# automl/RoBO

Measured on NVIDIA H100. Metric: EI evals/sec (GP N=4096, D=16, fp64), higher is better.
Workload: dtype f64

## Files before the change

robo_b200/csrc/gpk_api.cu:

```cuda
#include <algorithm>
#include <cmath>
#include <cstdarg>
#include <cstdio>
#include <cstring>
#include <cstdlib>
#include <dlfcn.h>
#include <string>
#include <vector>

#include "gpk_gemm.cuh"
#include "gpk_kernels.cuh"
#include "gpk_diag16.cuh"
#include "gpk_ozaki.cuh"
#include "gpk_de.cuh"
#include "gpk_lbfgs.cuh"
#include "gpk_cmaes.cuh"
#include "gpk_direct.cuh"
#include "gpk_es.cuh"
#include "gpk_esmc.cuh"
#include "gpk_rs.cuh"
#include "gpk_hyper.cuh"
#include "gpk_blr.cuh"
#include "gpk_rf.cuh"

// ... 7 lines not shown
    void* p = nullptr;
    size_t cap = 0;
};

}

struct gpk_handle {
    int device = 0;
    cudaStream_t stream = nullptr;
    cudaStream_t own_stream = nullptr;
    cudaStream_t side_stream = nullptr;
    std::vector<cudaEvent_t> ev_panel, ev_rest;
    int ozaki = 1;
    DevBuf oz_Pq, oz_Kq, oz_Kq2, oz_eP, oz_emax, oz_pmu2;
    int oz_last_variant = 0;
    int oz_cluster = 4;
    int oz_map_cs = 0;
    int oz_max_clusters[5] = {0, 0, 0, 0, 0};
    int oz_persist = 3;
    int oz_grid = 0;
    DevBuf oz_probe;
    long oz_linv_serial = -1;
    long linv_serial = 0;
    int oz_emax_host = 0;
    long oz_rows = 0, oz_rows2 = 0;
    CUtensorMap mapOzP, mapOzK, mapOzK2;
    double oz_launches = 0;
    int n_sm = 0;
    char err[1024] = {0};
    int loader = LOADER_TMA_WS;
    long chunk = 16384;
    bool chunk_user = false;
    int diag_prof = 0;
    DevBuf dprof;

    int n = 0, d = 0, NP = 0, nb = 0;
// ... 273 lines not shown
            attr[0].val.clusterDim.x = (unsigned)cs;
            attr[0].val.clusterDim.y = 1;
            attr[0].val.clusterDim.z = 1;
            cfg.attrs = attr;
            cfg.numAttrs = 1;
            int n = 0;
            CK(cudaOccupancyMaxActiveClusters(&n, gpk_oz_vargemm_kernel, &cfg));
            if (n < 1) { set_err(h, "no cluster of %d int8 contraction CTAs fits on this device", cs); return GPK_CUDA_ERROR; }
            h->oz_max_clusters[cs] = n;
        }
    }
    *out = h->oz_max_clusters[cs];
    return GPK_OK;
}

int launch_oz_contraction(gpk_handle* h, const CUtensorMap& mapP, const CUtensorMap& mapK, int nb, long rows_padded,
                          long NP, long rows, const int* eP, int eK, double* part_ssq, long ldpart) {
    OzArgs o;
    o.nb = nb; o.ncb = (int)(rows_padded / OZ_TN); o.NP = (int)NP; o.rows = (int)rows;
    const int cs = h->oz_cluster;
    o.group = (int)std::min<long>(512, std::max<long>(4, ((long)24 << 20) / ((long)OZ_TN * NP * OZ_S))) / cs * cs;
    o.eP = eP; o.eK = eK;
    o.part_ssq = part_ssq; o.ldpart = ldpart;
    const int persist = h->oz_persist == 3 ? (nb <= 32 ? 1 : 0) : h->oz_persist;
    const int tiles = o.nb * o.ncb;
    int grid = tiles;
    if (persist == 1) {
        int nclusters = 0, rc;
        if ((rc = oz_max_clusters(h, cs, &nclusters))) return rc;
        if (h->oz_grid > 0) nclusters = std::min(nclusters, h->oz_grid);
        grid = cs * std::min(tiles / cs, nclusters);
    }
    h->oz_last_variant = 1 + (persist == 1 ? 8 : 0) + (cs == 2 ? 16 : cs == 4 ? 32 : 0);
    CK(launch_oz(gpk_oz_vargemm_kernel, (unsigned)grid, cs, (size_t)OZ_SMEM, h->stream, mapP, mapK, o));
    CKL();
    return GPK_OK;
}

template <int EPI, int MI = 8>
int launch_gemm(gpk_handle* h, const CUtensorMap& mA, const CUtensorMap& mB, const GemmArgs& a, int njobs,
                cudaStream_t stream = nullptr, bool pdl = false) {
    if (njobs <= 0) return GPK_OK;
    if (stream == nullptr) stream = h->stream;
    if (pdl && h->loader != LOADER_CPASYNC && MI == 2) {
        CK(launch_pdl(gpk_gemm_nt_kernel<EPI, LOADER_TMA, MI>, dim3(njobs), dim3(GEMM_THREADS),
                      (size_t)gemm_smem_bytes(LOADER_TMA, MI), stream, mA, mB, a));
// ... 375 lines not shown
        const int lowest = -100000;
        CK(cudaMemcpyAsync(h->oz_emax.p, &lowest, 4, cudaMemcpyHostToDevice, h->stream));
        gpk_oz_rowexp_kernel<<<(unsigned)NP, 256, 0, h->stream>>>(ptr<double>(h->P), NP, (int)NP, ptr<int>(h->oz_eP), ptr<int>(h->oz_emax));
        CKL();
        gpk_oz_split_kernel<<<(unsigned)((NP * NP + 255) / 256), 256, 0, h->stream>>>(ptr<double>(h->P), NP, NP, ptr<int>(h->oz_eP), 0,
                                                                                   ptr<int8_t>(h->oz_Pq), NP * NP);
        CKL();
        if ((rc = ensure_alpha(h))) return rc;
        CK(cudaMemcpyAsync(&h->oz_emax_host, h->oz_emax.p, 4, cudaMemcpyDeviceToHost, h->stream));
        CK(cudaStreamSynchronize(h->stream));
        h->oz_map_cs = 0;
        h->oz_linv_serial = h->linv_serial;
    }
    if (h->oz_map_cs != h->oz_cluster) {
        int rc;
        if ((rc = make_oz_map(h, &h->mapOzP, h->oz_Pq.p, (long)OZ_S * NP, NP, OZ_TM / h->oz_cluster))) return rc;
        h->oz_map_cs = h->oz_cluster;
    }
    *usable = h->oz_emax_host <= OZ_MAX_EXP;
    return GPK_OK;
}

long chunk_rows(const gpk_handle* h) {
    if (h->chunk_user) return h->chunk;
    long c = ((1L << 26) / std::max(h->NP, 128)) / BM * BM;
    return std::min<long>(65536, std::max<long>(4096, c));
}

struct Feeder {
    virtual int ready(long lo, long hi, cudaStream_t st) = 0;
    virtual ~Feeder() {}
// ... 11 lines not shown
              long index_offset = 0, bool reset = true, long global_base = 0, Feeder* feeder = nullptr) {
    if (h->blr)
        return blr_score(h, dX, m, kind, eta, par, d_out, d_mu, d_var, d_best, d_nneg, index_offset, reset, global_base,
                         feeder);
    if (h->rf)
        return rf_score(h, dX, m, kind, eta, par, d_out, d_mu, d_var, d_best, d_nneg, index_offset, reset, global_base,
                        feeder);
    int rc = build_linv(h);
    if (rc) return rc;
    const long NP = h->NP;
    const long cap = std::min<long>(chunk_rows(h), round_up(std::max<long>(m, 1), BM));
    if ((rc = ensure_score_scratch(h, cap))) return rc;
    bool use_oz = false;
    if (m >= 2048 && (rc = prepare_ozaki(h, &use_oz))) return rc;
    int oz_eK = 0;
    if (use_oz) {
        if ((rc = ensure(h, h->oz_Kq, (size_t)OZ_S * cap * NP))) return rc;
        if (h->overlap && (rc = ensure(h, h->oz_Kq2, (size_t)OZ_S * cap * NP))) return rc;
        if ((rc = make_oz_map(h, &h->mapOzK, h->oz_Kq.p, (long)OZ_S * cap, NP, OZ_TN))) return rc;
        if (h->overlap && (rc = make_oz_map(h, &h->mapOzK2, h->oz_Kq2.p, (long)OZ_S * cap, NP, OZ_TN))) return rc;
        if (h->overlap && (rc = ensure(h, h->oz_pmu2, (size_t)h->nb * cap * 8))) return rc;
        oz_eK = oz_exponent(h->spec.amp);
    }
    if (d_best == nullptr) d_best = ptr<BestPair>(h->best);
    if (d_nneg == nullptr) d_nneg = ptr<unsigned long long>(h->nneg);
    if (reset) {
        CK(cudaMemsetAsync(d_best, 0xFF, sizeof(BestPair), h->stream));
        CK(cudaMemsetAsync(d_nneg, 0, 8, h->stream));
    }
    CK(cudaEventRecord(h->ev[6], h->stream));
    const int nchunks = (int)((m + cap - 1) / cap);
    const bool pipelined = h->overlap && nchunks > 1;
    if (pipelined) {
        while ((int)h->ev_cov.size() < nchunks) {
            cudaEvent_t e1, e2;
// ... 21 lines not shown
            if (frc) return frc;
        }
        const double* lo = h->has_bounds ? ptr<double>(h->lower) : nullptr;
        const double* up = h->has_bounds ? ptr<double>(h->upper) : nullptr;
        if (!use_oz)
            return launch_cov_tiles(h, st, train_operand(h), NP, h->n, dX + base * h->d, h->d, mc, mcp, lo, up,
                                    second ? ptr<double>(h->Kstar2) : ptr<double>(h->Kstar), NP, 0, small);
        CUtensorMap map;
        int mrc = make_cov_map(h, &map, (void*)train_operand(h), h->spec.n_terms, NP);
        if (mrc) return mrc;
        int8_t* qdst = second ? ptr<int8_t>(h->oz_Kq2) : ptr<int8_t>(h->oz_Kq);
        double* pmu = second ? ptr<double>(h->oz_pmu2) : ptr<double>(h->part_mu);
        const int gx = (int)(NP / 128);
        if (small)
            gpk_cov_oz_kernel<4><<<(unsigned)(gx * (mcp / 16)), 256, cov_oz_smem_bytes(h->spec.n_terms, 4), st>>>(
                map, h->spec, h->n, dX + base * h->d, h->d, mc, lo, up, ptr<double>(h->alpha), oz_eK, qdst, NP, cap * NP, pmu, cap, gx);
        else
            gpk_cov_oz_kernel<8><<<(unsigned)(gx * (mcp / 32)), 256, cov_oz_smem_bytes(h->spec.n_terms, 8), st>>>(
                map, h->spec, h->n, dX + base * h->d, h->d, mc, lo, up, ptr<double>(h->alpha), oz_eK, qdst, NP, cap * NP, pmu, cap, gx);
        CKL();
        return GPK_OK;
    };
    if (pipelined) {
        CK(cudaEventRecord(h->ev_order, h->stream));
        CK(cudaStreamWaitEvent(h->side_stream, h->ev_order, 0));
        if ((rc = launch_cov(0, h->side_stream, false))) return rc;
        CK(cudaEventRecord(h->ev_cov[0], h->side_stream));
    }
    for (int ci = 0; ci < nchunks; ++ci) {
        const long base = (long)ci * cap;
        const long mc = std::min(cap, m - base);
        const long mcp = round_up(mc, BM);
        const bool last = ci == nchunks - 1;
        if (last) CK(cudaEventRecord(h->ev[8], h->stream));
// ... 10 lines not shown
        const bool second = pipelined && (ci & 1);
        GemmArgs a;
        memset(&a, 0, sizeof(a));
        a.A = ptr<double>(h->P); a.lda = NP;
        a.B = second ? ptr<double>(h->Kstar2) : ptr<double>(h->Kstar); a.ldb = NP;
        a.alpha = 1.0;
        a.job_mode = JOBS_VARIANCE;
        a.nb = h->nb; a.mcb = (int)(mcp / BN);
        a.z = ptr<double>(h->Kbuf) + NP * NP;
        a.part_mu = ptr<double>(h->part_mu);
        a.part_ssq = ptr<double>(h->part_ssq);
        a.ldpart = cap;
        if (last) CK(cudaEventRecord(h->ev[10], h->stream));
        CK(cudaEventRecord(h->ev_g0[ci], h->stream));
        if (use_oz) {
            if ((rc = launch_oz_contraction(h, h->mapOzP, second ? h->mapOzK2 : h->mapOzK, h->nb, mcp, NP, cap,
                                            ptr<int>(h->oz_eP), oz_eK, a.part_ssq, a.ldpart)))
                return rc;
            h->oz_launches += 1;
        } else if ((rc = launch_gemm<EPI_COLREDUCE>(h, h->mapP, second ? h->mapKs2 : h->mapKs, a, h->nb * a.mcb))) return rc;
        CK(cudaEventRecord(h->ev_g1[ci], h->stream));
        if (last) CK(cudaEventRecord(h->ev[11], h->stream));
        if (pipelined && !use_oz) CK(cudaEventRecord(h->ev_gemm[ci], h->stream));
        h->launches_var += 1;
        h->last_chunk_rows = mcp;
        FinishArgs f;
        memset(&f, 0, sizeof(f));
        f.part_mu = ptr<double>(h->part_mu); f.part_ssq = ptr<double>(h->part_ssq);
        f.ldpart = cap; f.nparts = h->nb; f.m = mc; f.base = global_base + index_offset + base;
        f.kss = h->spec.amp; f.mean = h->mean;
        f.norm_out = h->norm_out; f.y_mean = h->y_mean; f.y_std = h->y_std;
// ... 381 lines not shown
    if (cudaMallocHost((void**)&h->pin, 64) != cudaSuccess) { delete h; return GPK_CUDA_ERROR; }
    if (get_encode_fn() == nullptr) h->loader = LOADER_CPASYNC;
    *out = h;
    return GPK_OK;
}

int gpk_destroy(gpk_handle* h) {
    if (!h) return GPK_OK;
    cudaSetDevice(h->device);
    cudaStreamSynchronize(h->stream);
    gpk_comm_destroy(h);
    if (h->ev_multi) cudaEventDestroy(h->ev_multi);
    DevBuf* bufs[] = {&h->Xrow, &h->Xt, &h->y, &h->Kbuf, &h->P, &h->Q, &h->W, &h->lower, &h->upper, &h->logdet_part,
                      &h->scal, &h->status, &h->jobs, &h->cand, &h->Kstar, &h->Kstar2, &h->cand2, &h->part_mu, &h->part_ssq, &h->out_mu,
                      &h->out_var, &h->out_acq, &h->block_best, &h->best, &h->nneg, &h->Vt, &h->cov, &h->XsT,
                      &h->tmpjobs, &h->alpha, &h->tmp1, &h->tmp2, &h->tmp3, &h->dprof, &h->Xts, &h->oz_Pq, &h->oz_Kq, &h->oz_Kq2, &h->oz_eP, &h->oz_emax, &h->oz_pmu2, &h->oz_probe,
                      &h->multi_cand, &h->multi_A, &h->multi_B, &h->multi_out, &h->multi_bb, &h->gather, &h->best_global,
                      &h->de_pop, &h->de_trial, &h->de_param, &h->de_E, &h->de_small, &h->de_sort, &h->lb_buf, &h->cma_buf, &h->dir_buf, &h->ep_buf, &h->es_state, &h->es_U, &h->es_work, &h->es_in, &h->mc_state, &h->mc_buf, &h->mc_stat, &h->fab_in, &h->rs_buf, &h->hy_buf,
                      &h->blr_data, &h->blr_post, &h->blr_work, &h->blr_bb,
                      &h->rf_data, &h->rf_work, &h->rf_nodes, &h->rf_bb};
    for (DevBuf* b : bufs)
        if (b->p) cudaFree(b->p);
    if (h->ev_ok)
        for (int i = 0; i < 16; ++i) cudaEventDestroy(h->ev[i]);
    if (h->ev_order) cudaEventDestroy(h->ev_order);
    for (int i = 0; i < 2; ++i)
        if (h->stage[i]) cudaFreeHost(h->stage[i]);
    for (cudaEvent_t e : h->ev_panel) cudaEventDestroy(e);
    for (cudaEvent_t e : h->ev_rest) cudaEventDestroy(e);
    for (cudaEvent_t e : h->ev_cov) cudaEventDestroy(e);
    for (cudaEvent_t e : h->ev_g0) cudaEventDestroy(e);
// ... 1471 lines not shown
    CK(cudaMemcpyAsync(z, ptr<double>(h->Kbuf) + (long)h->NP * h->NP, (size_t)h->n * 8, cudaMemcpyDeviceToHost, h->stream));
    CK(cudaStreamSynchronize(h->stream));
    return GPK_OK;
}

int gpk_oz_contract(gpk_handle* h, const double* P, int n, const double* Ks, long m, double amp, double* part_ssq,
                    int* eP, int* eK) {
    if (!h) return GPK_BAD_ARG;
    if (!P || !Ks || !part_ssq || !eP || !eK || n <= 0 || m <= 0 || !(amp > 0.0) || !std::isfinite(amp))
        BAD("gpk_oz_contract: bad arguments");
    const long NP = round_up(n, OZ_TM), MP = round_up(m, OZ_TM), nb = NP / OZ_TM;
    if (NP > 16384) BAD("gpk_oz_contract: n = %d pads to %ld > 16384 (the int32 level sums hold K <= 16384)", n, NP);
    for (long i = 0; i < m * (long)n; ++i)
        if (!(std::fabs(Ks[i]) <= amp)) BAD("gpk_oz_contract: |Ks| exceeds amp at entry %ld", i);
    CK(cudaSetDevice(h->device));
    const size_t oK = (size_t)NP * NP * 8, oPq = oK + (size_t)MP * NP * 8, oKq = oPq + (size_t)OZ_S * NP * NP;
    const size_t opart = oKq + (size_t)OZ_S * MP * NP, oe = opart + (size_t)nb * MP * 8, oemax = oe + (size_t)NP * 4;
    int rc;
    if ((rc = ensure(h, h->oz_probe, oemax + 4))) return rc;
    char* b = (char*)h->oz_probe.p;
    double* dP = (double*)b;
    double* dK = (double*)(b + oK);
    int8_t* dPq = (int8_t*)(b + oPq);
    int8_t* dKq = (int8_t*)(b + oKq);
    double* dpart = (double*)(b + opart);
    int* de = (int*)(b + oe);
    cudaStream_t st = h->stream;
    CK(cudaMemsetAsync(dP, 0, (size_t)NP * NP * 8, st));
    CK(cudaMemcpy2DAsync(dP, (size_t)NP * 8, P, (size_t)n * 8, (size_t)n * 8, (size_t)n, cudaMemcpyHostToDevice, st));
    CK(cudaMemsetAsync(dK, 0, (size_t)MP * NP * 8, st));
    CK(cudaMemcpy2DAsync(dK, (size_t)NP * 8, Ks, (size_t)n * 8, (size_t)n * 8, (size_t)m, cudaMemcpyHostToDevice, st));
    CK(cudaMemsetAsync(b + oemax, 0, 4, st));
    CK(cudaMemsetAsync(dpart, 0xFF, (size_t)nb * MP * 8, st));
    gpk_oz_rowexp_kernel<<<(unsigned)NP, 256, 0, st>>>(dP, NP, (int)NP, de, (int*)(b + oemax));
    CKL();
    gpk_oz_split_kernel<<<(unsigned)((NP * NP + 255) / 256), 256, 0, st>>>(dP, NP, NP, de, 0, dPq, NP * NP);
    CKL();
    const int ek = oz_exponent(amp);
    gpk_oz_split_kernel<<<(unsigned)((MP * NP + 255) / 256), 256, 0, st>>>(dK, MP, NP, nullptr, ek, dKq, MP * NP);
    CKL();
    CUtensorMap mapP, mapK;
    if ((rc = make_oz_map(h, &mapP, dPq, (long)OZ_S * NP, NP, OZ_TM / h->oz_cluster))) return rc;
    if ((rc = make_oz_map(h, &mapK, dKq, (long)OZ_S * MP, NP, OZ_TN))) return rc;
    if ((rc = launch_oz_contraction(h, mapP, mapK, (int)nb, MP, NP, MP, de, ek, dpart, MP))) return rc;
    CK(cudaMemcpy2DAsync(part_ssq, (size_t)m * 8, dpart, (size_t)MP * 8, (size_t)m * 8, (size_t)nb, cudaMemcpyDeviceToHost, st));
    CK(cudaMemcpyAsync(eP, de, (size_t)n * 4, cudaMemcpyDeviceToHost, st));
    CK(cudaStreamSynchronize(st));
    *eK = ek;
    return GPK_OK;
}

int gpk_ep_joint_min(gpk_handle* h, const double* mu, const double* V, int nb, double* logP, double* dlogPdMu,
                     double* dlogPdSigma, double* dlogPdMudMu, int* sweeps) {
    if (!h) return GPK_BAD_ARG;
    if (!mu || !V || !logP) BAD("gpk_ep_joint_min: need mu, V and logP");
    if (nb < 2 || nb > GPK_EP_MAX_NB) BAD("gpk_ep_joint_min: nb = %d outside 2 .. %d", nb, GPK_EP_MAX_NB);
    CK(cudaSetDevice(h->device));
    const size_t D = (size_t)nb, T = D * (D + 1) / 2;
    const size_t omu = 0, oV = omu + D, oP = oV + D * D, odM = oP + D, odMM = odM + D * D, odS = odMM + D * D * D;
// ... 370 lines not shown
```

robo_b200/csrc/gpk_ozaki.cuh:

```cuda
#pragma once
#include "gpk_gemm.cuh"

constexpr int OZ_S = 7;
constexpr int OZ_PAIRS = OZ_S * (OZ_S + 1) / 2;
constexpr int OZ_TM = 128, OZ_TN = 32;
constexpr int OZ_KB = 64;
constexpr int OZ_UK = 32;
constexpr int OZ_NSTG = 3;
constexpr int OZ_A_SLICE = OZ_TM * OZ_KB, OZ_B_SLICE = OZ_TN * OZ_KB;
constexpr int OZ_STAGE = OZ_S * (OZ_A_SLICE + OZ_B_SLICE);
constexpr int OZ_THREADS = 384;
constexpr int OZ_SMEM = OZ_NSTG * OZ_STAGE + 1024 + 256 + 2 * 8 * OZ_TN * 8;
constexpr int OZ_MAX_EXP = 7;

__host__ __device__ inline int oz_exponent(double amax) {
    if (!(amax > 0.0)) return 0;
    int ex;
    const double m = frexp(amax, &ex);
    return ex + 1 + (m * 128.0 >= 127.49 ? 1 : 0);
}
__device__ __forceinline__ unsigned long long oz_digits(double v) {
    const long long X = __double2ll_rn(v * 72057594037927936.0);
    return (unsigned long long)(X + 0x0080808080808080LL) ^ 0x0080808080808080ULL;
}
__device__ __forceinline__ int oz_digit_of(unsigned long long y, int s) { return (int)((y >> (8 * (OZ_S - 1 - s))) & 0xFFull); }

__device__ __forceinline__ void oz_mbar_wait(uint32_t bar, uint32_t parity) {
    while (!mbar_try_wait(bar, parity)) { }
// ... 22 lines not shown
    if (cs == 1) { mbar_arrive(bar); return; }
    uint32_t remote;
    asm volatile("mapa.shared::cluster.u32 %0, %1, %2;" : "=r"(remote) : "r"(bar), "r"(r));
    asm volatile("mbarrier.arrive.shared::cluster.b64 _, [%0];" :: "r"(remote) : "memory");
}
__device__ __forceinline__ uint64_t oz_desc(uint32_t smem_addr) {
    uint64_t d = 0;
    d |= (uint64_t)((smem_addr & 0x3FFFF) >> 4);
    d |= (uint64_t)1 << 16;
    d |= (uint64_t)(512 >> 4) << 32;
    d |= (uint64_t)2 << 62;
    return d;
}
#define OZ_ACC16(d) "+r"(d[0]), "+r"(d[1]), "+r"(d[2]), "+r"(d[3]), "+r"(d[4]), "+r"(d[5]), "+r"(d[6]), "+r"(d[7]), \
                    "+r"(d[8]), "+r"(d[9]), "+r"(d[10]), "+r"(d[11]), "+r"(d[12]), "+r"(d[13]), "+r"(d[14]), "+r"(d[15])
__device__ __forceinline__ void oz_wgmma_rs(uint32_t (&d)[16], const uint32_t (&a)[4], uint64_t b_desc) {
    asm volatile("wgmma.mma_async.sync.aligned.m64n32k32.s32.s8.s8 "
                 "{%0, %1, %2, %3, %4, %5, %6, %7, %8, %9, %10, %11, %12, %13, %14, %15}, {%16, %17, %18, %19}, %20, 1;"
                 : OZ_ACC16(d) : "r"(a[0]), "r"(a[1]), "r"(a[2]), "r"(a[3]), "l"(b_desc));
}
__device__ __forceinline__ void oz_lda_frag(uint32_t (&a)[2][4], uint32_t tile, int row0, int lane) {
    const int r = row0 + (lane & 7) + ((lane >> 3) & 1) * 8;
#pragma unroll
    for (int k = 0; k < OZ_KB / OZ_UK; ++k) {
        const int chunk = 2 * k + (lane >> 4);
        const uint32_t addr = tile + (uint32_t)(r * OZ_KB + ((chunk ^ ((r >> 1) & 3)) << 4));
        asm volatile("ldmatrix.sync.aligned.m8n8.x4.shared.b16 {%0, %1, %2, %3}, [%4];"
                     : "=r"(a[k][0]), "=r"(a[k][1]), "=r"(a[k][2]), "=r"(a[k][3]) : "r"(addr) : "memory");
    }
}
__device__ __forceinline__ void oz_wgmma_fence(uint32_t (&d)[16]) { asm volatile("" : OZ_ACC16(d) :: "memory"); }
__device__ __forceinline__ void wgmma_arrive() { asm volatile("wgmma.fence.sync.aligned;" ::: "memory"); }
__device__ __forceinline__ void wgmma_commit() { asm volatile("wgmma.commit_group.sync.aligned;" ::: "memory"); }
__device__ __forceinline__ void wgmma_wait_all() { asm volatile("wgmma.wait_group.sync.aligned 0;" ::: "memory"); }
__device__ __forceinline__ void wgmma_wait_one() { asm volatile("wgmma.wait_group.sync.aligned 1;" ::: "memory"); }

__device__ __forceinline__ double oz_i2d(uint32_t d) {
    return __hiloint2double(0x43300000, (int)(d ^ 0x80000000u)) - 4503601774854144.0;
}

__global__ void gpk_oz_rowexp_kernel(const double* __restrict__ A, long ld, int cols, int* __restrict__ e, int* __restrict__ emax) {
    const long r = blockIdx.x;
    double m = 0.0;
    for (int c = threadIdx.x; c < cols; c += 256) m = fmax(m, fabs(A[r * ld + c]));
    __shared__ double sh[256];
    sh[threadIdx.x] = m;
// ... 17 lines not shown
}

__device__ __forceinline__ void oz_tile_of(int id, int nb, int ncb, int group, int& ib, int& cb) {
    const int full = ncb / group;
    int grp = id / (nb * group), gsz = group;
    if (grp >= full) { grp = full; gsz = ncb - full * group; }
    id -= grp * nb * group;
    ib = nb - 1 - id / gsz;
    cb = grp * group + id % gsz;
}

struct OzArgs {
    int nb, ncb;
    int group;
    int NP, rows;
    const int* eP; int eK;
    double* part_ssq; long ldpart;
};

__global__ void __launch_bounds__(OZ_THREADS, 1)
gpk_oz_vargemm_kernel(const __grid_constant__ CUtensorMap mapP, const __grid_constant__ CUtensorMap mapK, const OzArgs g)
{
    extern __shared__ unsigned char oz_raw[];
    const uint32_t base = (smem_u32(oz_raw) + 1023u) & ~1023u;
    const uint32_t bar_full = base + OZ_NSTG * OZ_STAGE, bar_empty = bar_full + 8 * OZ_NSTG;
    const uint32_t red = base + OZ_NSTG * OZ_STAGE + 256;
    const int tid = threadIdx.x, wg = tid >> 7, lane = tid & 31;
    const uint32_t cs = oz_cluster_size(), rank = oz_cluster_rank();
    const int ncl = (int)(gridDim.x / cs), cid = (int)(blockIdx.x / cs);
    const int ncbc = g.ncb / (int)cs, gc = g.group / (int)cs;
    const int total = g.nb * ncbc;

    if (tid == 0) {
        for (int s = 0; s < OZ_NSTG; ++s) { mbar_init(bar_full + 8 * s, 1); mbar_init(bar_empty + 8 * s, 2 * cs); }
        fence_barrier_init();
        fence_proxy_async();
    }
    if (cs > 1) oz_cluster_sync(); else __syncthreads();

    if (wg == 0) {
        asm volatile("setmaxnreg.dec.sync.aligned.u32 40;" ::: "memory");
        if (tid == 0) {
            const int prow = OZ_TM / (int)cs;
            const uint16_t mask = (uint16_t)((1u << cs) - 1u);
            int it = 0;
            for (int t = cid; t < total; t += ncl) {
                int ib, cbc;
                oz_tile_of(t, g.nb, ncbc, gc, ib, cbc);
                const int cb = cbc * (int)cs + (int)rank;
                const int nkb = (ib + 1) * OZ_TM / OZ_KB;
                for (int kb = 0; kb < nkb; ++kb, ++it) {
                    const int s = it % OZ_NSTG;
                    if (it >= OZ_NSTG) oz_mbar_wait(bar_empty + 8 * s, (uint32_t)((it / OZ_NSTG - 1) & 1));
                    const uint32_t st = base + s * OZ_STAGE;
                    mbar_arrive_expect_tx(bar_full + 8 * s, OZ_STAGE);
#pragma unroll
                    for (int q = 0; q < OZ_S; ++q) {
                        const uint32_t pdst = st + q * OZ_A_SLICE + rank * prow * OZ_KB;
                        const int prow0 = q * g.NP + ib * OZ_TM + (int)rank * prow;
                        if (cs == 1) tma_load_2d(pdst, &mapP, kb * OZ_KB, prow0, bar_full + 8 * s);
                        else tma_load_2d_multicast(pdst, &mapP, kb * OZ_KB, prow0, bar_full + 8 * s, mask);
                        tma_load_2d(st + OZ_S * OZ_A_SLICE + q * OZ_B_SLICE, &mapK, kb * OZ_KB, q * g.rows + cb * OZ_TN,
                                    bar_full + 8 * s);
                    }
                }
            }
        }
        if (cs > 1) oz_cluster_sync();
        return;
    }
    asm volatile("setmaxnreg.inc.sync.aligned.u32 232;" ::: "memory");
    const int c = wg - 1, cw = (tid - 128) >> 5;
    const int r0 = c * 64 + (cw & 3) * 16 + (lane >> 2);
    int it = 0, tl = 0;
    for (int t = cid; t < total; t += ncl, ++tl) {
        int ib, cbc;
        oz_tile_of(t, g.nb, ncbc, gc, ib, cbc);
        const int cb = cbc * (int)cs + (int)rank;
        const int nkb = (ib + 1) * OZ_TM / OZ_KB;
        uint32_t acc[OZ_S][16];
#pragma unroll
        for (int l = 0; l < OZ_S; ++l)
#pragma unroll
            for (int e = 0; e < 16; ++e) acc[l][e] = 0u;
        uint32_t fa[2][2][4];
        for (int kb = 0; kb < nkb; kb += 2) {
#pragma unroll
            for (int h = 0; h < 2; ++h, ++it) {
                const int s = it % OZ_NSTG;
                oz_mbar_wait(bar_full + 8 * s, (uint32_t)((it / OZ_NSTG) & 1));
                const uint32_t st = base + s * OZ_STAGE;
#pragma unroll
                for (int a = 0; a < OZ_S; ++a) {
                    uint32_t (&f)[2][4] = fa[(h * OZ_S + a) & 1];
                    oz_lda_frag(f, st + a * OZ_A_SLICE, c * 64 + (cw & 3) * 16, lane);
                    wgmma_arrive();
#pragma unroll
                    for (int tk = 0; tk < OZ_S - a; ++tk)
#pragma unroll
                        for (int k = 0; k < OZ_KB / OZ_UK; ++k)
                            oz_wgmma_rs(acc[a + tk], f[k], oz_desc(st + OZ_S * OZ_A_SLICE + tk * OZ_B_SLICE + k * OZ_UK));
                    wgmma_commit();
                    wgmma_wait_one();
                    if (a == 0 && (h == 1 || kb > 0) && (uint32_t)(tid & 127) < cs)
                        oz_release_stage(bar_empty + 8 * ((it + OZ_NSTG - 1) % OZ_NSTG), cs, (uint32_t)(tid & 127));
                }
            }
        }
        wgmma_wait_all();
#pragma unroll
        for (int l = 0; l < OZ_S; ++l) oz_wgmma_fence(acc[l]);
        if ((uint32_t)(tid & 127) < cs) oz_release_stage(bar_empty + 8 * ((it + OZ_NSTG - 1) % OZ_NSTG), cs, (uint32_t)(tid & 127));
        const double rs0 = ldexp(1.0, g.eP[ib * OZ_TM + r0] + g.eK), rs1 = ldexp(1.0, g.eP[ib * OZ_TM + r0 + 8] + g.eK);
        double col[8];
#pragma unroll
        for (int j = 0; j < 8; ++j) col[j] = 0.0;
#pragma unroll
        for (int e = 0; e < 16; ++e) {
            double v = 0.0;
#pragma unroll
            for (int lvl = OZ_S - 1; lvl >= 0; --lvl) v = fma(oz_i2d(acc[lvl][e]), ldexp(1.0, -8 * (lvl + 2)), v);
            const double x = v * (((e >> 1) & 1) ? rs1 : rs0);
            col[2 * (e >> 2) + (e & 1)] += x * x;
        }
#pragma unroll
        for (int j = 0; j < 8; ++j)
#pragma unroll
            for (int o = 4; o < 32; o <<= 1) col[j] += __shfl_xor_sync(0xffffffffu, col[j], o);
        const uint32_t redt = red + (uint32_t)((tl & 1) * 8 * OZ_TN * 8);
        if (lane < 4) {
#pragma unroll
            for (int j = 0; j < 8; ++j) sts64(redt + (uint32_t)((cw * OZ_TN + 8 * (j >> 1) + 2 * lane + (j & 1)) * 8), col[j]);
        }
        named_bar_sync(1, 256);
        const int et = tid - 128;
        if (et < OZ_TN) {
            double s2 = 0.0;
#pragma unroll
            for (int w8 = 0; w8 < 8; ++w8) s2 += lds64(redt + (uint32_t)((w8 * OZ_TN + et) * 8));
            g.part_ssq[(long)ib * g.ldpart + cb * OZ_TN + et] = s2;
        }
    }
    if (cs > 1) oz_cluster_sync();
}

template <int CC, bool DIGITS = true>
__global__ void __launch_bounds__(256, CC == 8 ? 2 : 4)
gpk_cov_oz_kernel(const __grid_constant__ CUtensorMap mapX, const KSpec ks, int n,
                  const double* __restrict__ cand, int dc, long m,
                  const double* __restrict__ lower, const double* __restrict__ upper,
                  const double* __restrict__ alpha, int eK, int8_t* __restrict__ Kq, long ldq, long slice_stride,
                  double* __restrict__ part_mu, long ldpart, int gx)
{
    constexpr int TC = 4 * CC;
    extern __shared__ unsigned char cov_raw[];
// ... 151 lines not shown
```

Measured before the change: 2.656 million.

## Restructure int8 Ozaki contraction with wider N tiles, level split across warpgroups, dynamic scheduling

Reworks the int8 Ozaki contraction kernel so each tile uses m64n96 WGMMA with 64-row A halves instead of m64n32 with 128 rows. The two consumer warpgroups now split the seven slice levels between them and hand partial sums through a shared-memory slab. A dynamic tile counter replaces the static stride, and the default cluster size drops from 4 to 1. K buffers are padded and zeroed to a multiple of 4*TN. The aim is higher tensor-core throughput and better load balance. The cost is more register pressure, extra named-barrier handoffs between warpgroups, and loss of multicast sharing of P tiles.

New measurement: 2.821 million (median of 6 runs). 1.06x the previous value.

```diff
diff --git a/robo_b200/csrc/gpk_api.cu b/robo_b200/csrc/gpk_api.cu
--- a/robo_b200/csrc/gpk_api.cu
+++ b/robo_b200/csrc/gpk_api.cu
@@ -45,12 +45,13 @@
     int ozaki = 1;
     DevBuf oz_Pq, oz_Kq, oz_Kq2, oz_eP, oz_emax, oz_pmu2;
     int oz_last_variant = 0;
-    int oz_cluster = 4;
+    int oz_cluster = 1;
     int oz_map_cs = 0;
     int oz_max_clusters[5] = {0, 0, 0, 0, 0};
     int oz_persist = 3;
     int oz_grid = 0;
     DevBuf oz_probe;
+    DevBuf oz_next;
     long oz_linv_serial = -1;
     long linv_serial = 0;
     int oz_emax_host = 0;
@@ -354,15 +355,17 @@
     return GPK_OK;
 }
 
-int launch_oz_contraction(gpk_handle* h, const CUtensorMap& mapP, const CUtensorMap& mapK, int nb, long rows_padded,
+int launch_oz_contraction(gpk_handle* h, const CUtensorMap& mapP, const CUtensorMap& mapK, int nb, long cols,
                           long NP, long rows, const int* eP, int eK, double* part_ssq, long ldpart) {
+    const int cs = h->oz_cluster;
     OzArgs o;
-    o.nb = nb; o.ncb = (int)(rows_padded / OZ_TN); o.NP = (int)NP; o.rows = (int)rows;
-    const int cs = h->oz_cluster;
+    o.nb = nb; o.ncb = (int)((cols + (long)OZ_TN * cs - 1) / ((long)OZ_TN * cs)) * cs; o.NP = (int)NP; o.rows = (int)rows;
+    o.cols = (int)cols;
     o.group = (int)std::min<long>(512, std::max<long>(4, ((long)24 << 20) / ((long)OZ_TN * NP * OZ_S))) / cs * cs;
     o.eP = eP; o.eK = eK;
     o.part_ssq = part_ssq; o.ldpart = ldpart;
-    const int persist = h->oz_persist == 3 ? (nb <= 32 ? 1 : 0) : h->oz_persist;
+    o.next = nullptr;
+    const int persist = h->oz_persist == 3 ? (nb <= 12 ? 1 : 0) : h->oz_persist;
     const int tiles = o.nb * o.ncb;
     int grid = tiles;
     if (persist == 1) {
@@ -370,6 +373,12 @@
         if ((rc = oz_max_clusters(h, cs, &nclusters))) return rc;
         if (h->oz_grid > 0) nclusters = std::min(nclusters, h->oz_grid);
         grid = cs * std::min(tiles / cs, nclusters);
+        if (cs == 1) {
+            int rc2;
+            if ((rc2 = ensure(h, h->oz_next, 4))) return rc2;
+            CK(cudaMemsetAsync(h->oz_next.p, 0, 4, h->stream));
+            o.next = ptr<int>(h->oz_next);
+        }
     }
     h->oz_last_variant = 1 + (persist == 1 ? 8 : 0) + (cs == 2 ? 16 : cs == 4 ? 32 : 0);
     CK(launch_oz(gpk_oz_vargemm_kernel, (unsigned)grid, cs, (size_t)OZ_SMEM, h->stream, mapP, mapK, o));
@@ -775,7 +784,7 @@
     }
     if (h->oz_map_cs != h->oz_cluster) {
         int rc;
-        if ((rc = make_oz_map(h, &h->mapOzP, h->oz_Pq.p, (long)OZ_S * NP, NP, OZ_TM / h->oz_cluster))) return rc;
+        if ((rc = make_oz_map(h, &h->mapOzP, h->oz_Pq.p, (long)OZ_S * NP, NP, OZ_HM / h->oz_cluster))) return rc;
         h->oz_map_cs = h->oz_cluster;
     }
     *usable = h->oz_emax_host <= OZ_MAX_EXP;
@@ -817,11 +826,16 @@
     bool use_oz = false;
     if (m >= 2048 && (rc = prepare_ozaki(h, &use_oz))) return rc;
     int oz_eK = 0;
+    const long capq = round_up(cap, OZ_KPAD);
     if (use_oz) {
-        if ((rc = ensure(h, h->oz_Kq, (size_t)OZ_S * cap * NP))) return rc;
-        if (h->overlap && (rc = ensure(h, h->oz_Kq2, (size_t)OZ_S * cap * NP))) return rc;
-        if ((rc = make_oz_map(h, &h->mapOzK, h->oz_Kq.p, (long)OZ_S * cap, NP, OZ_TN))) return rc;
-        if (h->overlap && (rc = make_oz_map(h, &h->mapOzK2, h->oz_Kq2.p, (long)OZ_S * cap, NP, OZ_TN))) return rc;
+        for (DevBuf* q : {&h->oz_Kq, &h->oz_Kq2}) {
+            if (q == &h->oz_Kq2 && !h->overlap) continue;
+            bool grew = false;
+            if ((rc = ensure(h, *q, (size_t)OZ_S * capq * NP, &grew))) return rc;
+            if (grew) CK(cudaMemsetAsync(q->p, 0, (size_t)OZ_S * capq * NP, h->stream));
+        }
+        if ((rc = make_oz_map(h, &h->mapOzK, h->oz_Kq.p, (long)OZ_S * capq, NP, OZ_TN))) return rc;
+        if (h->overlap && (rc = make_oz_map(h, &h->mapOzK2, h->oz_Kq2.p, (long)OZ_S * capq, NP, OZ_TN))) return rc;
         if (h->overlap && (rc = ensure(h, h->oz_pmu2, (size_t)h->nb * cap * 8))) return rc;
         oz_eK = oz_exponent(h->spec.amp);
     }
@@ -873,10 +887,10 @@
         const int gx = (int)(NP / 128);
         if (small)
             gpk_cov_oz_kernel<4><<<(unsigned)(gx * (mcp / 16)), 256, cov_oz_smem_bytes(h->spec.n_terms, 4), st>>>(
-                map, h->spec, h->n, dX + base * h->d, h->d, mc, lo, up, ptr<double>(h->alpha), oz_eK, qdst, NP, cap * NP, pmu, cap, gx);
+                map, h->spec, h->n, dX + base * h->d, h->d, mc, lo, up, ptr<double>(h->alpha), oz_eK, qdst, NP, capq * NP, pmu, cap, gx);
         else
             gpk_cov_oz_kernel<8><<<(unsigned)(gx * (mcp / 32)), 256, cov_oz_smem_bytes(h->spec.n_terms, 8), st>>>(
-                map, h->spec, h->n, dX + base * h->d, h->d, mc, lo, up, ptr<double>(h->alpha), oz_eK, qdst, NP, cap * NP, pmu, cap, gx);
+                map, h->spec, h->n, dX + base * h->d, h->d, mc, lo, up, ptr<double>(h->alpha), oz_eK, qdst, NP, capq * NP, pmu, cap, gx);
         CKL();
         return GPK_OK;
     };
@@ -917,7 +931,7 @@
         if (last) CK(cudaEventRecord(h->ev[10], h->stream));
         CK(cudaEventRecord(h->ev_g0[ci], h->stream));
         if (use_oz) {
-            if ((rc = launch_oz_contraction(h, h->mapOzP, second ? h->mapOzK2 : h->mapOzK, h->nb, mcp, NP, cap,
+            if ((rc = launch_oz_contraction(h, h->mapOzP, second ? h->mapOzK2 : h->mapOzK, h->nb, mcp, NP, capq,
                                             ptr<int>(h->oz_eP), oz_eK, a.part_ssq, a.ldpart)))
                 return rc;
             h->oz_launches += 1;
@@ -1329,7 +1343,7 @@
     DevBuf* bufs[] = {&h->Xrow, &h->Xt, &h->y, &h->Kbuf, &h->P, &h->Q, &h->W, &h->lower, &h->upper, &h->logdet_part,
                       &h->scal, &h->status, &h->jobs, &h->cand, &h->Kstar, &h->Kstar2, &h->cand2, &h->part_mu, &h->part_ssq, &h->out_mu,
                       &h->out_var, &h->out_acq, &h->block_best, &h->best, &h->nneg, &h->Vt, &h->cov, &h->XsT,
-                      &h->tmpjobs, &h->alpha, &h->tmp1, &h->tmp2, &h->tmp3, &h->dprof, &h->Xts, &h->oz_Pq, &h->oz_Kq, &h->oz_Kq2, &h->oz_eP, &h->oz_emax, &h->oz_pmu2, &h->oz_probe,
+                      &h->tmpjobs, &h->alpha, &h->tmp1, &h->tmp2, &h->tmp3, &h->dprof, &h->Xts, &h->oz_Pq, &h->oz_Kq, &h->oz_Kq2, &h->oz_eP, &h->oz_emax, &h->oz_pmu2, &h->oz_probe, &h->oz_next,
                       &h->multi_cand, &h->multi_A, &h->multi_B, &h->multi_out, &h->multi_bb, &h->gather, &h->best_global,
                       &h->de_pop, &h->de_trial, &h->de_param, &h->de_E, &h->de_small, &h->de_sort, &h->lb_buf, &h->cma_buf, &h->dir_buf, &h->ep_buf, &h->es_state, &h->es_U, &h->es_work, &h->es_in, &h->mc_state, &h->mc_buf, &h->mc_stat, &h->fab_in, &h->rs_buf, &h->hy_buf,
                       &h->blr_data, &h->blr_post, &h->blr_work, &h->blr_bb,
@@ -2831,8 +2845,9 @@
     for (long i = 0; i < m * (long)n; ++i)
         if (!(std::fabs(Ks[i]) <= amp)) BAD("gpk_oz_contract: |Ks| exceeds amp at entry %ld", i);
     CK(cudaSetDevice(h->device));
+    const long MQ = round_up(MP, OZ_KPAD);
     const size_t oK = (size_t)NP * NP * 8, oPq = oK + (size_t)MP * NP * 8, oKq = oPq + (size_t)OZ_S * NP * NP;
-    const size_t opart = oKq + (size_t)OZ_S * MP * NP, oe = opart + (size_t)nb * MP * 8, oemax = oe + (size_t)NP * 4;
+    const size_t opart = oKq + (size_t)OZ_S * MQ * NP, oe = opart + (size_t)nb * MP * 8, oemax = oe + (size_t)NP * 4;
     int rc;
     if ((rc = ensure(h, h->oz_probe, oemax + 4))) return rc;
     char* b = (char*)h->oz_probe.p;
@@ -2854,12 +2869,13 @@
     gpk_oz_split_kernel<<<(unsigned)((NP * NP + 255) / 256), 256, 0, st>>>(dP, NP, NP, de, 0, dPq, NP * NP);
     CKL();
     const int ek = oz_exponent(amp);
-    gpk_oz_split_kernel<<<(unsigned)((MP * NP + 255) / 256), 256, 0, st>>>(dK, MP, NP, nullptr, ek, dKq, MP * NP);
+    CK(cudaMemsetAsync(dKq, 0, (size_t)OZ_S * MQ * NP, st));
+    gpk_oz_split_kernel<<<(unsigned)((MP * NP + 255) / 256), 256, 0, st>>>(dK, MP, NP, nullptr, ek, dKq, MQ * NP);
     CKL();
     CUtensorMap mapP, mapK;
-    if ((rc = make_oz_map(h, &mapP, dPq, (long)OZ_S * NP, NP, OZ_TM / h->oz_cluster))) return rc;
-    if ((rc = make_oz_map(h, &mapK, dKq, (long)OZ_S * MP, NP, OZ_TN))) return rc;
-    if ((rc = launch_oz_contraction(h, mapP, mapK, (int)nb, MP, NP, MP, de, ek, dpart, MP))) return rc;
+    if ((rc = make_oz_map(h, &mapP, dPq, (long)OZ_S * NP, NP, OZ_HM / h->oz_cluster))) return rc;
+    if ((rc = make_oz_map(h, &mapK, dKq, (long)OZ_S * MQ, NP, OZ_TN))) return rc;
+    if ((rc = launch_oz_contraction(h, mapP, mapK, (int)nb, MP, NP, MQ, de, ek, dpart, MP))) return rc;
     CK(cudaMemcpy2DAsync(part_ssq, (size_t)m * 8, dpart, (size_t)MP * 8, (size_t)m * 8, (size_t)nb, cudaMemcpyDeviceToHost, st));
     CK(cudaMemcpyAsync(eP, de, (size_t)n * 4, cudaMemcpyDeviceToHost, st));
     CK(cudaStreamSynchronize(st));
diff --git a/robo_b200/csrc/gpk_ozaki.cuh b/robo_b200/csrc/gpk_ozaki.cuh
--- a/robo_b200/csrc/gpk_ozaki.cuh
+++ b/robo_b200/csrc/gpk_ozaki.cuh
@@ -3,15 +3,22 @@
 
 constexpr int OZ_S = 7;
 constexpr int OZ_PAIRS = OZ_S * (OZ_S + 1) / 2;
-constexpr int OZ_TM = 128, OZ_TN = 32;
+constexpr int OZ_TM = 128, OZ_HM = 64, OZ_TN = 96;
+constexpr int OZ_LSPLIT = 4;
+constexpr int OZ_NACC = OZ_TN / 2;
+constexpr int OZ_KPAD = 4 * OZ_TN;
 constexpr int OZ_KB = 64;
 constexpr int OZ_UK = 32;
 constexpr int OZ_NSTG = 3;
-constexpr int OZ_A_SLICE = OZ_TM * OZ_KB, OZ_B_SLICE = OZ_TN * OZ_KB;
+constexpr int OZ_A_SLICE = OZ_HM * OZ_KB, OZ_B_SLICE = OZ_TN * OZ_KB;
 constexpr int OZ_STAGE = OZ_S * (OZ_A_SLICE + OZ_B_SLICE);
 constexpr int OZ_THREADS = 384;
-constexpr int OZ_SMEM = OZ_NSTG * OZ_STAGE + 1024 + 256 + 2 * 8 * OZ_TN * 8;
+constexpr int OZ_RED = 4 * OZ_TN * 8;
+constexpr int OZ_SLAB = 128 * 4 * 8;
+constexpr int OZ_SMEM = OZ_NSTG * OZ_STAGE + 1024 + 256 + 2 * OZ_RED + 2 * OZ_SLAB;
 constexpr int OZ_MAX_EXP = 7;
+constexpr int OZ_NTILE = 4;
+static_assert(OZ_SMEM <= 227 * 1024, "int8 contraction: shared memory");
 
 __host__ __device__ inline int oz_exponent(double amax) {
     if (!(amax > 0.0)) return 0;
@@ -64,10 +71,17 @@
 }
 #define OZ_ACC16(d) "+r"(d[0]), "+r"(d[1]), "+r"(d[2]), "+r"(d[3]), "+r"(d[4]), "+r"(d[5]), "+r"(d[6]), "+r"(d[7]), \
                     "+r"(d[8]), "+r"(d[9]), "+r"(d[10]), "+r"(d[11]), "+r"(d[12]), "+r"(d[13]), "+r"(d[14]), "+r"(d[15])
-__device__ __forceinline__ void oz_wgmma_rs(uint32_t (&d)[16], const uint32_t (&a)[4], uint64_t b_desc) {
-    asm volatile("wgmma.mma_async.sync.aligned.m64n32k32.s32.s8.s8 "
-                 "{%0, %1, %2, %3, %4, %5, %6, %7, %8, %9, %10, %11, %12, %13, %14, %15}, {%16, %17, %18, %19}, %20, 1;"
-                 : OZ_ACC16(d) : "r"(a[0]), "r"(a[1]), "r"(a[2]), "r"(a[3]), "l"(b_desc));
+__device__ __forceinline__ void oz_wgmma_rs(uint32_t (&d)[OZ_NACC], const uint32_t (&a)[4], uint64_t b_desc) {
+    asm volatile("wgmma.mma_async.sync.aligned.m64n96k32.s32.s8.s8 "
+                 "{%0, %1, %2, %3, %4, %5, %6, %7, %8, %9, %10, %11, %12, %13, %14, %15, %16, %17, %18, %19, %20, %21, %22, "
+                 "%23, %24, %25, %26, %27, %28, %29, %30, %31, %32, %33, %34, %35, %36, %37, %38, %39, %40, %41, %42, %43, %44, "
+                 "%45, %46, %47}, {%48, %49, %50, %51}, %52, 1;"
+                 : OZ_ACC16(d), "+r"(d[16]), "+r"(d[17]), "+r"(d[18]), "+r"(d[19]), "+r"(d[20]), "+r"(d[21]), "+r"(d[22]),
+                   "+r"(d[23]), "+r"(d[24]), "+r"(d[25]), "+r"(d[26]), "+r"(d[27]), "+r"(d[28]), "+r"(d[29]), "+r"(d[30]),
+                   "+r"(d[31]), "+r"(d[32]), "+r"(d[33]), "+r"(d[34]), "+r"(d[35]), "+r"(d[36]), "+r"(d[37]), "+r"(d[38]),
+                   "+r"(d[39]), "+r"(d[40]), "+r"(d[41]), "+r"(d[42]), "+r"(d[43]), "+r"(d[44]), "+r"(d[45]), "+r"(d[46]),
+                   "+r"(d[47])
+                 : "r"(a[0]), "r"(a[1]), "r"(a[2]), "r"(a[3]), "l"(b_desc));
 }
 __device__ __forceinline__ void oz_lda_frag(uint32_t (&a)[2][4], uint32_t tile, int row0, int lane) {
     const int r = row0 + (lane & 7) + ((lane >> 3) & 1) * 8;
@@ -80,6 +94,13 @@
     }
 }
 __device__ __forceinline__ void oz_wgmma_fence(uint32_t (&d)[16]) { asm volatile("" : OZ_ACC16(d) :: "memory"); }
+__device__ __forceinline__ void oz_wgmma_fence(uint32_t (&d)[OZ_NACC]) {
+#pragma unroll
+    for (int i = 0; i < OZ_NACC; i += 16) oz_wgmma_fence(*reinterpret_cast<uint32_t(*)[16]>(d + i));
+}
+__device__ __forceinline__ void oz_bar_arrive(int id, int nthreads) {
+    asm volatile("bar.arrive %0, %1;" :: "r"(id), "r"(nthreads) : "memory");
+}
 __device__ __forceinline__ void wgmma_arrive() { asm volatile("wgmma.fence.sync.aligned;" ::: "memory"); }
 __device__ __forceinline__ void wgmma_commit() { asm volatile("wgmma.commit_group.sync.aligned;" ::: "memory"); }
 __device__ __forceinline__ void wgmma_wait_all() { asm volatile("wgmma.wait_group.sync.aligned 0;" ::: "memory"); }
@@ -127,9 +148,65 @@
     int nb, ncb;
     int group;
     int NP, rows;
+    int cols;
+    int* next;
     const int* eP; int eK;
     double* part_ssq; long ldpart;
 };
+
+template <int LO, int HI, int H>
+__device__ __forceinline__ void oz_consume_stage(uint32_t (&acc)[HI - LO + 1][OZ_NACC], uint32_t (&fa)[2][2][4], int& it,
+                                                 bool release, uint32_t base, uint32_t bar_full, uint32_t bar_empty,
+                                                 int row0, int lane, uint32_t cs, uint32_t t127) {
+    const int s = it % OZ_NSTG;
+    oz_mbar_wait(bar_full + 8 * s, (uint32_t)((it / OZ_NSTG) & 1));
+    const uint32_t st = base + s * OZ_STAGE;
+#pragma unroll
+    for (int a = 0; a <= HI; ++a) {
+        uint32_t (&f)[2][4] = fa[(H * (HI + 1) + a) & 1];
+        oz_lda_frag(f, st + a * OZ_A_SLICE, row0, lane);
+        wgmma_arrive();
+#pragma unroll
+        for (int t = (LO > a ? LO - a : 0); t <= HI - a; ++t)
+#pragma unroll
+            for (int k = 0; k < OZ_KB / OZ_UK; ++k)
+                oz_wgmma_rs(acc[a + t - LO], f[k], oz_desc(st + OZ_S * OZ_A_SLICE + t * OZ_B_SLICE + k * OZ_UK));
+        wgmma_commit();
+        wgmma_wait_one();
+        if (a == 0 && release && t127 < cs) oz_release_stage(bar_empty + 8 * ((it + OZ_NSTG - 1) % OZ_NSTG), cs, t127);
+    }
+    ++it;
+}
+template <int LO, int HI>
+__device__ __forceinline__ void oz_consume_pass(uint32_t (&acc)[HI - LO + 1][OZ_NACC], int nkb, int& it, uint32_t base,
+                                                uint32_t bar_full, uint32_t bar_empty, int row0, int lane, uint32_t cs,
+                                                uint32_t t127) {
+#pragma unroll
+    for (int l = 0; l <= HI - LO; ++l)
+#pragma unroll
+        for (int e = 0; e < OZ_NACC; ++e) acc[l][e] = 0u;
+    uint32_t fa[2][2][4];
+    int kb = 0;
+    for (; kb + 1 < nkb; kb += 2) {
+        oz_consume_stage<LO, HI, 0>(acc, fa, it, kb > 0, base, bar_full, bar_empty, row0, lane, cs, t127);
+        oz_consume_stage<LO, HI, 1>(acc, fa, it, true, base, bar_full, bar_empty, row0, lane, cs, t127);
+    }
+    if (kb < nkb) oz_consume_stage<LO, HI, 0>(acc, fa, it, kb > 0, base, bar_full, bar_empty, row0, lane, cs, t127);
+    wgmma_wait_all();
+#pragma unroll
+    for (int l = 0; l <= HI - LO; ++l) oz_wgmma_fence(acc[l]);
+    if (t127 < cs) oz_release_stage(bar_empty + 8 * ((it + OZ_NSTG - 1) % OZ_NSTG), cs, t127);
+}
+
+__device__ __forceinline__ int oz_next_tile(int n, uint32_t tile_full, uint32_t tile_empty, uint32_t tile_slot, int lane) {
+    const int j = n % OZ_NTILE;
+    oz_mbar_wait(tile_full + 8 * j, (uint32_t)((n / OZ_NTILE) & 1));
+    int t;
+    asm volatile("ld.shared.u32 %0, [%1];" : "=r"(t) : "r"(tile_slot + 4 * j) : "memory");
+    __syncwarp();
+    if (lane == 0) mbar_arrive(tile_empty + 8 * j);
+    return t;
+}
 
 __global__ void __launch_bounds__(OZ_THREADS, 1)
 gpk_oz_vargemm_kernel(const __grid_constant__ CUtensorMap mapP, const __grid_constant__ CUtensorMap mapK, const OzArgs g)
@@ -137,7 +214,10 @@
     extern __shared__ unsigned char oz_raw[];
     const uint32_t base = (smem_u32(oz_raw) + 1023u) & ~1023u;
     const uint32_t bar_full = base + OZ_NSTG * OZ_STAGE, bar_empty = bar_full + 8 * OZ_NSTG;
+    const uint32_t tile_full = bar_empty + 8 * OZ_NSTG, tile_empty = tile_full + 8 * OZ_NTILE, tile_slot = tile_empty + 8 * OZ_NTILE;
     const uint32_t red = base + OZ_NSTG * OZ_STAGE + 256;
+    const uint32_t slab = red + 2 * OZ_RED;
+    constexpr int OZ_BAR_RED = 1, OZ_BAR_FULL = 2, OZ_BAR_EMPTY = 4;
     const int tid = threadIdx.x, wg = tid >> 7, lane = tid & 31;
     const uint32_t cs = oz_cluster_size(), rank = oz_cluster_rank();
     const int ncl = (int)(gridDim.x / cs), cid = (int)(blockIdx.x / cs);
@@ -146,6 +226,7 @@
 
     if (tid == 0) {
         for (int s = 0; s < OZ_NSTG; ++s) { mbar_init(bar_full + 8 * s, 1); mbar_init(bar_empty + 8 * s, 2 * cs); }
+        for (int j = 0; j < OZ_NTILE; ++j) { mbar_init(tile_full + 8 * j, 1); mbar_init(tile_empty + 8 * j, 8); }
         fence_barrier_init();
         fence_proxy_async();
     }
@@ -154,27 +235,35 @@
     if (wg == 0) {
         asm volatile("setmaxnreg.dec.sync.aligned.u32 40;" ::: "memory");
         if (tid == 0) {
-            const int prow = OZ_TM / (int)cs;
+            const int prow = OZ_HM / (int)cs;
             const uint16_t mask = (uint16_t)((1u << cs) - 1u);
             int it = 0;
-            for (int t = cid; t < total; t += ncl) {
+            for (int n = 0;; ++n) {
+                const int j = n % OZ_NTILE;
+                if (n >= OZ_NTILE) oz_mbar_wait(tile_empty + 8 * j, (uint32_t)((n / OZ_NTILE - 1) & 1));
+                const int t = g.next ? atomicAdd(g.next, 1) : cid + n * ncl;
+                asm volatile("st.shared.u32 [%0], %1;" :: "r"(tile_slot + 4 * j), "r"(t) : "memory");
+                mbar_arrive(tile_full + 8 * j);
+                if (t >= total) break;
                 int ib, cbc;
                 oz_tile_of(t, g.nb, ncbc, gc, ib, cbc);
                 const int cb = cbc * (int)cs + (int)rank;
-                const int nkb = (ib + 1) * OZ_TM / OZ_KB;
-                for (int kb = 0; kb < nkb; ++kb, ++it) {
-                    const int s = it % OZ_NSTG;
-                    if (it >= OZ_NSTG) oz_mbar_wait(bar_empty + 8 * s, (uint32_t)((it / OZ_NSTG - 1) & 1));
-                    const uint32_t st = base + s * OZ_STAGE;
-                    mbar_arrive_expect_tx(bar_full + 8 * s, OZ_STAGE);
-#pragma unroll
-                    for (int q = 0; q < OZ_S; ++q) {
-                        const uint32_t pdst = st + q * OZ_A_SLICE + rank * prow * OZ_KB;
-                        const int prow0 = q * g.NP + ib * OZ_TM + (int)rank * prow;
-                        if (cs == 1) tma_load_2d(pdst, &mapP, kb * OZ_KB, prow0, bar_full + 8 * s);
-                        else tma_load_2d_multicast(pdst, &mapP, kb * OZ_KB, prow0, bar_full + 8 * s, mask);
-                        tma_load_2d(st + OZ_S * OZ_A_SLICE + q * OZ_B_SLICE, &mapK, kb * OZ_KB, q * g.rows + cb * OZ_TN,
-                                    bar_full + 8 * s);
+                for (int p = 0; p < 2; ++p) {
+                    const int nkb = 2 * ib + 1 + p;
+                    const int arow = ib * OZ_TM + p * OZ_HM + (int)rank * prow;
+                    for (int kb = 0; kb < nkb; ++kb, ++it) {
+                        const int s = it % OZ_NSTG;
+                        if (it >= OZ_NSTG) oz_mbar_wait(bar_empty + 8 * s, (uint32_t)((it / OZ_NSTG - 1) & 1));
+                        const uint32_t st = base + s * OZ_STAGE;
+                        mbar_arrive_expect_tx(bar_full + 8 * s, OZ_STAGE);
+#pragma unroll
+                        for (int q = 0; q < OZ_S; ++q) {
+                            const uint32_t pdst = st + q * OZ_A_SLICE + rank * prow * OZ_KB;
+                            if (cs == 1) tma_load_2d(pdst, &mapP, kb * OZ_KB, q * g.NP + arow, bar_full + 8 * s);
+                            else tma_load_2d_multicast(pdst, &mapP, kb * OZ_KB, q * g.NP + arow, bar_full + 8 * s, mask);
+                            tma_load_2d(st + OZ_S * OZ_A_SLICE + q * OZ_B_SLICE, &mapK, kb * OZ_KB, q * g.rows + cb * OZ_TN,
+                                        bar_full + 8 * s);
+                        }
                     }
                 }
             }
@@ -182,76 +271,93 @@
         if (cs > 1) oz_cluster_sync();
         return;
     }
-    asm volatile("setmaxnreg.inc.sync.aligned.u32 232;" ::: "memory");
-    const int c = wg - 1, cw = (tid - 128) >> 5;
-    const int r0 = c * 64 + (cw & 3) * 16 + (lane >> 2);
-    int it = 0, tl = 0;
-    for (int t = cid; t < total; t += ncl, ++tl) {
-        int ib, cbc;
-        oz_tile_of(t, g.nb, ncbc, gc, ib, cbc);
-        const int cb = cbc * (int)cs + (int)rank;
-        const int nkb = (ib + 1) * OZ_TM / OZ_KB;
-        uint32_t acc[OZ_S][16];
-#pragma unroll
-        for (int l = 0; l < OZ_S; ++l)
-#pragma unroll
-            for (int e = 0; e < 16; ++e) acc[l][e] = 0u;
-        uint32_t fa[2][2][4];
-        for (int kb = 0; kb < nkb; kb += 2) {
-#pragma unroll
-            for (int h = 0; h < 2; ++h, ++it) {
-                const int s = it % OZ_NSTG;
-                oz_mbar_wait(bar_full + 8 * s, (uint32_t)((it / OZ_NSTG) & 1));
-                const uint32_t st = base + s * OZ_STAGE;
-#pragma unroll
-                for (int a = 0; a < OZ_S; ++a) {
-                    uint32_t (&f)[2][4] = fa[(h * OZ_S + a) & 1];
-                    oz_lda_frag(f, st + a * OZ_A_SLICE, c * 64 + (cw & 3) * 16, lane);
-                    wgmma_arrive();
-#pragma unroll
-                    for (int tk = 0; tk < OZ_S - a; ++tk)
-#pragma unroll
-                        for (int k = 0; k < OZ_KB / OZ_UK; ++k)
-                            oz_wgmma_rs(acc[a + tk], f[k], oz_desc(st + OZ_S * OZ_A_SLICE + tk * OZ_B_SLICE + k * OZ_UK));
-                    wgmma_commit();
-                    wgmma_wait_one();
-                    if (a == 0 && (h == 1 || kb > 0) && (uint32_t)(tid & 127) < cs)
-                        oz_release_stage(bar_empty + 8 * ((it + OZ_NSTG - 1) % OZ_NSTG), cs, (uint32_t)(tid & 127));
+    const int w4 = (tid >> 5) & 3;
+    const uint32_t t127 = (uint32_t)(tid & 127);
+    const int row0 = w4 * 16;
+    int it = 0;
+    if (wg == 2) {
+        asm volatile("setmaxnreg.inc.sync.aligned.u32 208;" ::: "memory");
+        for (int n = 0;; ++n) {
+            const int t = oz_next_tile(n, tile_full, tile_empty, tile_slot, lane);
+            if (t >= total) break;
+            int ib, cbc;
+            oz_tile_of(t, g.nb, ncbc, gc, ib, cbc);
+            for (int p = 0; p < 2; ++p) {
+                uint32_t acc[OZ_S - OZ_LSPLIT][OZ_NACC];
+                oz_consume_pass<OZ_LSPLIT, OZ_S - 1>(acc, 2 * ib + 1 + p, it, base, bar_full, bar_empty, row0, lane, cs, t127);
+#pragma unroll
+                for (int j = 0; j < OZ_TN / 8; ++j) {
+                    double v[4];
+#pragma unroll
+                    for (int i = 0; i < 4; ++i) {
+                        v[i] = 0.0;
+#pragma unroll
+                        for (int lvl = OZ_S - 1; lvl >= OZ_LSPLIT; --lvl)
+                            v[i] = fma(oz_i2d(acc[lvl - OZ_LSPLIT][4 * j + i]), ldexp(1.0, -8 * (lvl + 2)), v[i]);
+                    }
+                    const uint32_t sl = slab + (uint32_t)((j & 1) * OZ_SLAB) + t127 * 8u;
+                    named_bar_sync(OZ_BAR_EMPTY + (j & 1), 256);
+#pragma unroll
+                    for (int i = 0; i < 4; ++i) sts64(sl + 1024u * i, v[i]);
+                    oz_bar_arrive(OZ_BAR_FULL + (j & 1), 256);
                 }
             }
         }
-        wgmma_wait_all();
-#pragma unroll
-        for (int l = 0; l < OZ_S; ++l) oz_wgmma_fence(acc[l]);
-        if ((uint32_t)(tid & 127) < cs) oz_release_stage(bar_empty + 8 * ((it + OZ_NSTG - 1) % OZ_NSTG), cs, (uint32_t)(tid & 127));
-        const double rs0 = ldexp(1.0, g.eP[ib * OZ_TM + r0] + g.eK), rs1 = ldexp(1.0, g.eP[ib * OZ_TM + r0 + 8] + g.eK);
-        double col[8];
-#pragma unroll
-        for (int j = 0; j < 8; ++j) col[j] = 0.0;
-#pragma unroll
-        for (int e = 0; e < 16; ++e) {
-            double v = 0.0;
-#pragma unroll
-            for (int lvl = OZ_S - 1; lvl >= 0; --lvl) v = fma(oz_i2d(acc[lvl][e]), ldexp(1.0, -8 * (lvl + 2)), v);
-            const double x = v * (((e >> 1) & 1) ? rs1 : rs0);
-            col[2 * (e >> 2) + (e & 1)] += x * x;
-        }
-#pragma unroll
-        for (int j = 0; j < 8; ++j)
-#pragma unroll
-            for (int o = 4; o < 32; o <<= 1) col[j] += __shfl_xor_sync(0xffffffffu, col[j], o);
-        const uint32_t redt = red + (uint32_t)((tl & 1) * 8 * OZ_TN * 8);
-        if (lane < 4) {
-#pragma unroll
-            for (int j = 0; j < 8; ++j) sts64(redt + (uint32_t)((cw * OZ_TN + 8 * (j >> 1) + 2 * lane + (j & 1)) * 8), col[j]);
-        }
-        named_bar_sync(1, 256);
-        const int et = tid - 128;
-        if (et < OZ_TN) {
-            double s2 = 0.0;
-#pragma unroll
-            for (int w8 = 0; w8 < 8; ++w8) s2 += lds64(redt + (uint32_t)((w8 * OZ_TN + et) * 8));
-            g.part_ssq[(long)ib * g.ldpart + cb * OZ_TN + et] = s2;
+        named_bar_sync(OZ_BAR_EMPTY, 256);
+        named_bar_sync(OZ_BAR_EMPTY + 1, 256);
+    } else {
+        asm volatile("setmaxnreg.inc.sync.aligned.u32 256;" ::: "memory");
+        oz_bar_arrive(OZ_BAR_EMPTY, 256);
+        oz_bar_arrive(OZ_BAR_EMPTY + 1, 256);
+        double carry = 0.0;
+        int pc = 0;
+        for (int n = 0;; ++n) {
+            const int t = oz_next_tile(n, tile_full, tile_empty, tile_slot, lane);
+            if (t >= total) break;
+            int ib, cbc;
+            oz_tile_of(t, g.nb, ncbc, gc, ib, cbc);
+            const int cb = cbc * (int)cs + (int)rank;
+            for (int p = 0; p < 2; ++p, ++pc) {
+                uint32_t acc[OZ_LSPLIT][OZ_NACC];
+                oz_consume_pass<0, OZ_LSPLIT - 1>(acc, 2 * ib + 1 + p, it, base, bar_full, bar_empty, row0, lane, cs, t127);
+                const int r = ib * OZ_TM + p * OZ_HM + row0 + (lane >> 2);
+                const double rs0 = ldexp(1.0, g.eP[r] + g.eK), rs1 = ldexp(1.0, g.eP[r + 8] + g.eK);
+                const uint32_t redt = red + (uint32_t)((pc & 1) * OZ_RED);
+#pragma unroll
+                for (int j = 0; j < OZ_TN / 8; ++j) {
+                    const uint32_t sl = slab + (uint32_t)((j & 1) * OZ_SLAB) + t127 * 8u;
+                    double x[4];
+                    named_bar_sync(OZ_BAR_FULL + (j & 1), 256);
+#pragma unroll
+                    for (int i = 0; i < 4; ++i) x[i] = lds64(sl + 1024u * i);
+                    oz_bar_arrive(OZ_BAR_EMPTY + (j & 1), 256);
+#pragma unroll
+                    for (int i = 0; i < 4; ++i) {
+                        double v = x[i];
+#pragma unroll
+                        for (int lvl = OZ_LSPLIT - 1; lvl >= 0; --lvl) v = fma(oz_i2d(acc[lvl][4 * j + i]), ldexp(1.0, -8 * (lvl + 2)), v);
+                        x[i] = v * ((i >> 1) ? rs1 : rs0);
+                    }
+                    double col[2] = {fma(x[2], x[2], x[0] * x[0]), fma(x[3], x[3], x[1] * x[1])};
+#pragma unroll
+                    for (int h = 0; h < 2; ++h)
+#pragma unroll
+                        for (int o = 4; o < 32; o <<= 1) col[h] += __shfl_xor_sync(0xffffffffu, col[h], o);
+                    if (lane < 4) {
+                        sts64(redt + (uint32_t)((w4 * OZ_TN + 8 * j + 2 * lane) * 8), col[0]);
+                        sts64(redt + (uint32_t)((w4 * OZ_TN + 8 * j + 2 * lane + 1) * 8), col[1]);
+                    }
+                }
+                named_bar_sync(OZ_BAR_RED, 128);
+                if (t127 < (uint32_t)OZ_TN) {
+                    double s2 = p == 0 ? 0.0 : carry;
+#pragma unroll
+                    for (int w = 0; w < 4; ++w) s2 += lds64(redt + (uint32_t)((w * OZ_TN + (int)t127) * 8));
+                    const int c = cb * OZ_TN + (int)t127;
+                    if (p == 0) carry = s2;
+                    else if (c < g.cols) g.part_ssq[(long)ib * g.ldpart + c] = s2;
+                }
+            }
         }
     }
     if (cs > 1) oz_cluster_sync();
```
